# ParBLiSS/kmerind

Hardware: AMD Instinct MI355X
Metric: kmers_per_sec_indexed (higher is better)
Workload: dtype u64

## Files before the change

kmerind_amd/csrc/kmi_front.h:

```cpp
#pragma once
#include "kmi_front_bytes.h"

namespace kmi {

constexpr int kFrWaves = 4, kFrThreads = kFrWaves * kWave;
constexpr uint32_t kFrRing = 256;
constexpr uint32_t kFrRunQ = 256;
constexpr uint32_t kFrStep = 4096;
constexpr uint32_t kFrRowDw = 12;
constexpr uint32_t kFrNone = 0xffu;
constexpr uint32_t kFrOverrun = 256u << 10;

struct FrRange { uint32_t l0, n_lines, n_runs, n_items; };
struct __attribute__((packed, aligned(1))) FrU4 { uint32_t x, y, z, w; };

template <int W> struct FrCfg {
  static constexpr int SEG = W >= 19 ? 127 : (W >= 13 ? 80 : (W >= 11 ? 64 : 44));
  static constexpr int KMAX = W >= 19 ? 32 : (W >= 13 ? 28 : (W >= 11 ? 22 : 20));
  static constexpr int ND = (SEG + KMAX - 1 + 3) / 4;
  static constexpr int NR = (ND + 3) / 4;
};

__device__ __forceinline__ uint32_t pack_dna4(uint32_t w, uint32_t *ok_out = nullptr) {
  const uint32_t x = w & 0xDFDFDFDFu;
  const uint32_t idx = (x >> 1) & 0x03030303u;
  const uint32_t expect = byte_perm(0u, 0x47544341u, idx);
  const uint32_t ok = zero_bytes(x ^ expect);
  if (ok_out) *ok_out = ok;
  const uint32_t lut = byte_perm(0u, 0x01000203u, idx);
  const uint32_t v1 = ok >> 7, vm = v1 | (v1 << 1);
  const uint32_t cc = (lut & vm) | (0x03030303u & ~vm);
  const uint32_t p1 = cc | (cc >> 6);
  return (p1 | (p1 >> 12)) & 0xFFu;
}

__device__ __forceinline__ uint32_t dna4_ok(uint32_t w) {
  const uint32_t x = w & 0xDFDFDFDFu;
  const uint32_t idx = (x >> 1) & 0x03030303u;
  return zero_bytes(x ^ byte_perm(0u, 0x47544341u, idx));
}

#if defined(KMI_FR_TIMING) && !defined(KMI_FR_LEAVE)
#define KMI_FR_LEAVE
#endif
#ifdef KMI_FR_LEAVE
constexpr uint32_t kFrTimingWaves = 16384;
__device__ unsigned long long g_fr_wave_clock[2 * kFrTimingWaves];
#endif

template <int W, bool EDGES = false>
__global__ __launch_bounds__(kFrThreads) void sk_front_kernel(const uint8_t *__restrict__ bytes, uint64_t n_bytes, uint64_t range_bytes, uint32_t n_ranges,
                                                             uint32_t k, bool rna, uint32_t run_cap, uint32_t item_cap, uint32_t ranges_per_group,
                                                             FrRange *__restrict__ info, uint32_t *__restrict__ run_items, uint32_t *__restrict__ rows,
                                                             uint32_t *__restrict__ items, uint32_t *__restrict__ wg_hist,
                                                             unsigned long long *__restrict__ n_windows, uint32_t *__restrict__ flags,
                                                             uint32_t r_first = 0u, uint32_t r_end = 0xffffffffu, uint32_t *__restrict__ queue = nullptr) {
  constexpr bool edges = EDGES;
  if (r_end > n_ranges) r_end = n_ranges;
  using F = FrCfg<W>;
  constexpr int CAP = kSkListCap;
  constexpr uint32_t INF = 0xffffffffu, RM = kFrRing - 1u, QM = kFrRunQ - 1u;
  __shared__ uint32_t s_S[kFrWaves][kFrRing], s_E[kFrWaves][kFrRing], s_rq[kFrWaves][kFrRunQ];
  __shared__ uint32_t s_list[kFrWaves][(CAP + 2) * kWave];
  __shared__ uint32_t s_hist[kFrWaves][kNumCoarse];
  const uint32_t lane = lane_id(), wv = wave_id();
  uint32_t *const S = s_S[wv], *const E = s_E[wv], *const rq = s_rq[wv], *const list = s_list[wv], *const hist = s_hist[wv];
  auto wave_sync = [&]() { asm volatile("s_waitcnt lgkmcnt(0)" ::: "memory"); __builtin_amdgcn_wave_barrier(); };
  const uint32_t m = k - (uint32_t)W + 1u;
  const uint32_t mmask = (m >= 16u) ? 0xffffffffu : ((1u << (2u * m)) - 1u);
  const uint32_t topsh = 2u * m - 2u;
  const uint32_t nmax = sk_nmax_of(k) - (edges ? kSkEdgeWindows : 0u);
  const uint32_t seg = (uint32_t)F::SEG;
  const uint32_t n_waves = gridDim.x * (uint32_t)kFrWaves;
#ifdef KMI_FR_LEAVE
  const unsigned long long t_enter = wall_clock64();
#endif
#ifdef KMI_FR_TIMING
  unsigned long long acc[8] = {0, 0, 0, 0, 0, 0, 0, 0}, tq = clock64();
#define FQ_MARK(i) { const unsigned long long now_ = clock64(); acc[i] += now_ - tq; tq = now_; }
#else
#define FQ_MARK(i)
#endif
  for (uint32_t r = r_first + blockIdx.x * (uint32_t)kFrWaves + wv; r < r_end;) {
    const uint64_t B = (uint64_t)r * range_bytes;
    const uint32_t len = (uint32_t)((n_bytes - B < range_bytes) ? (n_bytes - B) : range_bytes);
    for (uint32_t i = lane; i < (uint32_t)kNumCoarse; i += kWave) hist[i] = 0;
    uint32_t why = 0; bool bail = false;
    uint32_t q_next = 0;
    if (queue && lane == 0) q_next = atomicAdd(queue, 1u);
    uint32_t carry = (B == 0) ? 1u : (is_eol((uint32_t)__builtin_amdgcn_readfirstlane((int)bytes[B - 1])) ? 1u : 0u);
    const uint32_t r_next = queue ? r_first + n_waves + (uint32_t)__builtin_amdgcn_readfirstlane((int)q_next) : r + n_waves;
    const uint32_t eoff = carry ? 0u : 1u;
    uint32_t n_starts = 0, n_ends = 0, n_owned = 0, done = 0, l0 = (r == 0) ? 0u : INF;
    if (r == 0 && __builtin_amdgcn_readfirstlane((int)bytes[0]) != (int)'@') { why |= 2u; bail = true; }
    uint32_t rq_head = 0, rq_tail = 0, run_count = 0, item_count = 0;
    unsigned long long windows = 0;
    uint32_t p = 0;
    bool producing = true;
    FrU4 n0, n1, n2, n3;
    n0.x = n0.y = n0.z = n0.w = 0; n1 = n0; n2 = n0; n3 = n0;
    if (B + 64ull * lane + 64 <= n_bytes) {
      const uint8_t *q = bytes + B + 64ull * lane;
      n0 = *reinterpret_cast<const FrU4 *>(q); n1 = *reinterpret_cast<const FrU4 *>(q + 16);
      n2 = *reinterpret_cast<const FrU4 *>(q + 32); n3 = *reinterpret_cast<const FrU4 *>(q + 48);
    }
    uint32_t mk_ch = 0, mk_want = 0;
    auto eol32 = [](const FrU4 &a, const FrU4 &b) -> uint32_t {
      uint32_t d0 = __builtin_amdgcn_udot4(eol_flags(a.x), 0x08040201u, 0u, false);
      d0 = __builtin_amdgcn_udot4(eol_flags(a.y), 0x80402010u, d0, false);
      uint32_t d1 = __builtin_amdgcn_udot4(eol_flags(a.z), 0x08040201u, 0u, false);
      d1 = __builtin_amdgcn_udot4(eol_flags(a.w), 0x80402010u, d1, false);
      uint32_t d2 = __builtin_amdgcn_udot4(eol_flags(b.x), 0x08040201u, 0u, false);
      d2 = __builtin_amdgcn_udot4(eol_flags(b.y), 0x80402010u, d2, false);
      uint32_t d3 = __builtin_amdgcn_udot4(eol_flags(b.z), 0x08040201u, 0u, false);
      d3 = __builtin_amdgcn_udot4(eol_flags(b.w), 0x80402010u, d3, false);
      return (d0 >> 7) | (d1 << 1) | (d2 << 9) | (d3 << 17);
    };
    while (!bail) {
      while (producing && rq_tail - rq_head < (uint32_t)kWave && !bail) {
        const uint64_t g = B + p + 64ull * lane;
        uint32_t eol_lo = 0, eol_hi = 0;
        const FrU4 v0 = n0, v1 = n1, v2 = n2, v3 = n3;
        {
          const uint64_t gn = g + kFrStep;
          if (gn + 64 <= n_bytes) {
            const uint8_t *q = bytes + gn;
            n0 = *reinterpret_cast<const FrU4 *>(q); n1 = *reinterpret_cast<const FrU4 *>(q + 16);
            n2 = *reinterpret_cast<const FrU4 *>(q + 32); n3 = *reinterpret_cast<const FrU4 *>(q + 48);
          }
        }
        FQ_MARK(0)
        if (g + 64 <= n_bytes) {
          eol_lo = eol32(v0, v1); eol_hi = eol32(v2, v3);
        } else {
#pragma unroll 1
          for (uint32_t i = 0; i < 64u; ++i) {
            const bool e = (g + i >= n_bytes) || is_eol(bytes[g + i]);
            if (i < 32u) eol_lo |= (e ? 1u : 0u) << i; else eol_hi |= (e ? 1u : 0u) << (i - 32u);
          }
        }
        FQ_MARK(1)
        const uint32_t prev = (uint32_t)__builtin_amdgcn_update_dpp((int)carry, (int)(eol_hi >> 31), 0x138 , 0xf, 0xf, false);
        const uint32_t before_lo = (eol_lo << 1) | prev, before_hi = (eol_hi << 1) | (eol_lo >> 31);
        uint32_t ls_lo = ~eol_lo & before_lo, ls_hi = ~eol_hi & before_hi, le_lo = eol_lo & ~before_lo, le_hi = eol_hi & ~before_hi;
        const uint32_t base = p + 64u * lane;
        const uint32_t ns = (uint32_t)__builtin_popcount(ls_lo) + (uint32_t)__builtin_popcount(ls_hi);
        const uint32_t ne = (uint32_t)__builtin_popcount(le_lo) + (uint32_t)__builtin_popcount(le_hi);
        if (__any(ns > 8u || ne > 8u)) { why |= 4u; bail = true; break; }
        const uint32_t no = base < len ? ns : 0u;
        const uint32_t packed = ns | (ne << 10) | (no << 20);
        const uint32_t inc = wave_inclusive_sum_dpp(packed);
        const uint32_t tot = __builtin_amdgcn_readlane(inc, kWave - 1);
        const uint32_t NS = tot & 1023u, NE = (tot >> 10) & 1023u, NO = tot >> 20;
        if (NS > kFrRing / 2u || NE > kFrRing / 2u) { why |= 4u; bail = true; break; }
        uint32_t rs = n_starts + ((inc - packed) & 1023u), re = n_ends + (((inc - packed) >> 10) & 1023u);
        while (ls_lo) { S[rs & RM] = base + (uint32_t)__builtin_ctz(ls_lo); ++rs; ls_lo &= ls_lo - 1u; }
        while (ls_hi) { S[rs & RM] = base + 32u + (uint32_t)__builtin_ctz(ls_hi); ++rs; ls_hi &= ls_hi - 1u; }
        while (le_lo) { E[re & RM] = base + (uint32_t)__builtin_ctz(le_lo); ++re; le_lo &= le_lo - 1u; }
        while (le_hi) { E[re & RM] = base + 32u + (uint32_t)__builtin_ctz(le_hi); ++re; le_hi &= le_hi - 1u; }
        n_starts += NS; n_ends += NE; n_owned += NO;
        carry = (uint32_t)__builtin_amdgcn_readlane(eol_hi, kWave - 1) >> 31;
        p += kFrStep;
        if (p > len + kFrOverrun) { why |= 32u; bail = true; break; }
        const bool at_eof = B + p > n_bytes;
        wave_sync();
        if (l0 == INF && n_starts > 0u) {
          if ((uint32_t)__builtin_amdgcn_readfirstlane((int)S[0]) >= len) l0 = kFrNone;
          else if (at_eof && n_starts < 6u) {
            l0 = (0u - n_starts) & 3u;
          } else if (n_starts >= 6u) {
            const uint32_t nl = 6u;
            uint32_t c = 0;
            if (lane < nl) c = bytes[B + S[lane]];
            const uint32_t c2 = __shfl_down(c, 2, kWave);
            const bool cand = lane < 4u && lane + 2u < nl && c == (uint32_t)'@' && c2 == (uint32_t)'+';
            const unsigned long long cm = __ballot(cand);
            if (__popcll(cm) != 1) { why |= 8u; bail = true; break; }
            l0 = (4u - (uint32_t)__builtin_ctzll(cm)) & 3u;
          }
        }
        if (l0 == kFrNone) { producing = false; break; }
        if (l0 != INF) {
          const uint32_t complete = n_ends >= eoff ? (n_starts < n_ends - eoff ? n_starts : n_ends - eoff) : 0u;
          for (uint32_t j0 = done; j0 < complete && !bail; j0 += kWave) {
            const uint32_t j = j0 + lane;
            const bool have = j < complete;
            uint32_t sj = 0, L = 0, role = 4;
            if (have) { sj = S[j & RM]; L = E[(j + eoff) & RM] - sj; role = (l0 + j) & 3u; }
            const bool owned = have && sj < len;
            bool bad = false;
            if (mk_want && mk_ch != mk_want) bad = true;
            mk_want = 0;
            if (owned && (role == 0u || role == 2u)) { mk_ch = bytes[B + sj]; mk_want = role == 0u ? (uint32_t)'@' : (uint32_t)'+'; }
            if (have && role == 3u && j >= 2u && S[(j - 2u) & RM] < len) bad = bad || (E[(j - 2u + eoff) & RM] - S[(j - 2u) & RM] != L);
            if (__any(bad)) {
              why |= 16u; bail = true; break;
            }
            uint32_t nr = 0, nwin = 0;
            if (owned && role == 1u && L >= k) { nwin = L - k + 1u; nr = (nwin + seg - 1u) / seg; }
            const uint32_t rinc = wave_inclusive_sum_dpp(nr);
            const uint32_t rtot = __builtin_amdgcn_readlane(rinc, kWave - 1);
            if ((rq_tail + rtot - rq_head > kFrRunQ || __any(have && (sj >> 24))) && rtot) { { why |= 32u; bail = true; break; } }
            uint32_t o = rq_tail + rinc - nr;
            for (uint32_t i = 0; i < nr; ++i) {
              const uint32_t left = nwin - i * seg;
              rq[(o + i) & QM] = (sj + i * seg) | (((left < seg ? left : seg) - 1u) << 24);
            }
            rq_tail += rtot;
          }
          if (bail) break;
          done = complete;
          if (at_eof || (p >= len && complete >= n_owned + 2u)) producing = false;
        } else if (at_eof) { producing = false; }
        wave_sync();
      }
      if (bail) break;
      FQ_MARK(2)
      const uint32_t avail = rq_tail - rq_head;
      if (avail == 0u) { if (!producing) break; continue; }
      const uint32_t take = avail < (uint32_t)kWave ? avail : (uint32_t)kWave;
      const bool mine = lane < take;
      const uint32_t rv = mine ? rq[(rq_head + lane) & QM] : 0u;
      rq_head += take;
      if (run_count + take > run_cap) { why |= 64u; bail = true; break; }
      const uint32_t L = mine ? (rv >> 24) + 1u : 0u;
      const uint64_t g0 = B + (rv & 0xffffffu);
      {
        const uint32_t wsum = __builtin_amdgcn_readlane(wave_inclusive_sum_dpp(L), kWave - 1);
        windows += wsum;
      }
      uint32_t rw[16];
#pragma unroll
      for (int i = 0; i < 16; ++i) rw[i] = 0;
      uint32_t other = 0;
      auto pack_exact = [&]() {
#pragma unroll
        for (int q = 0; q < F::NR; ++q) {
          FrU4 v = *reinterpret_cast<const FrU4 *>(bytes + g0 + 16 * q);
          if (rna) { v.x = swap_tu_dword(v.x); v.y = swap_tu_dword(v.y); v.z = swap_tu_dword(v.z); v.w = swap_tu_dword(v.w); }
          uint32_t okd[4];
          rw[q] = pack_dna4(v.x, &okd[0]) | (pack_dna4(v.y, &okd[1]) << 8) | (pack_dna4(v.z, &okd[2]) << 16) | (pack_dna4(v.w, &okd[3]) << 24);
          if (edges) {
            const uint32_t nbits = 8u * (L + k - 1u);
#pragma unroll
            for (int e = 0; e < 4; ++e) {
              const uint32_t at = 8u * (16u * (uint32_t)q + 4u * (uint32_t)e);
              const uint32_t vm = nbits >= at + 32u ? 0x80808080u : (nbits <= at ? 0u : (0x80808080u & ((1u << (nbits - at)) - 1u)));
              other |= ~okd[e] & vm;
            }
          }
        }
      };
      constexpr bool fast_pack = !edges;
      const bool whole = mine && g0 + 16ull * F::NR <= n_bytes;
      if (fast_pack) {
        uint32_t bad = 0;
        if (whole) {
          const uint32_t nb = L + k - 1u;
#pragma unroll
          for (int q = 0; q < F::NR; ++q) {
            FrU4 v = *reinterpret_cast<const FrU4 *>(bytes + g0 + 16 * q);
            if (rna) { v.x = swap_tu_dword(v.x); v.y = swap_tu_dword(v.y); v.z = swap_tu_dword(v.z); v.w = swap_tu_dword(v.w); }
            uint32_t d = 0;
            const uint32_t c0 = pack_codes4(v.x, d), c1 = pack_codes4(v.y, d), c2 = pack_codes4(v.z, d), c3 = pack_codes4(v.w, d);
            rw[q] = c0 | (c1 << 8) | (c2 << 16) | (c3 << 24);
            bad |= (16u * (uint32_t)(q + 1) <= nb) ? d : 0u;
          }
          const uint32_t rem = nb & 15u, qt = nb >> 4;
          if (rem) {
            FrU4 v = *reinterpret_cast<const FrU4 *>(bytes + g0 + 16u * qt);
            if (rna) { v.x = swap_tu_dword(v.x); v.y = swap_tu_dword(v.y); v.z = swap_tu_dword(v.z); v.w = swap_tu_dword(v.w); }
            bad |= dna4_other_in_first(v.x, rem) | dna4_other_in_first(v.y, rem > 4u ? rem - 4u : 0u) |
                   dna4_other_in_first(v.z, rem > 8u ? rem - 8u : 0u) | dna4_other_in_first(v.w, rem > 12u ? rem - 12u : 0u);
          }
          bad &= 0xDFDFDFDFu;
        }
        if (__any(bad != 0u)) { if (whole) pack_exact(); }
      } else if (whole) pack_exact();
      if (mine && !whole) {
        const uint32_t nb = L + k - 1u;
#pragma unroll 1
        for (uint32_t i = 0; i < nb; ++i) {
          uint32_t c = bytes[g0 + i];
          if (rna) c = swap_tu_dword(c) & 0xffu;
          const uint32_t code = pack_dna4(c | 0x0A0A0A00u) & 3u;
          if (edges) other |= ~dna4_ok(c | 0x41414100u) & 0x80u;
          const uint32_t wi = i >> 4, sh = (i & 15u) * 2u;
#pragma unroll
          for (int q = 0; q < F::NR; ++q) rw[q] |= (wi == (uint32_t)q) ? (code << sh) : 0u;
        }
      }
      if (edges) {
        if (mine) {
          const uint32_t nb = L + k - 1u;
          uint32_t lb = bytes[g0 - 1u], rb = g0 + nb < n_bytes ? (uint32_t)bytes[g0 + nb] : (uint32_t)'\n';
          if (rna) { lb = swap_tu_dword(lb) & 0xffu; rb = swap_tu_dword(rb) & 0xffu; }
          const uint32_t lc = is_eol(lb) ? 0u : 4u - (pack_dna4(lb | 0x0A0A0A00u) & 3u), rc = is_eol(rb) ? 0u : 4u - (pack_dna4(rb | 0x0A0A0A00u) & 3u);
          if (!is_eol(lb)) other |= ~dna4_ok(lb | 0x41414100u) & 0x80u;
          if (!is_eol(rb)) other |= ~dna4_ok(rb | 0x41414100u) & 0x80u;
          rw[kFrRowDw - 1] = lc | (rc << 3);
        }
        if (__any(other != 0u)) { why |= 1024u; bail = true; break; }
      }
      FQ_MARK(3)
      if (mine) {
        const uint64_t ri = (uint64_t)r * run_cap + run_count + lane;
        uint4 *rp = reinterpret_cast<uint4 *>(rows + ri * kFrRowDw);
        rp[0] = make_uint4(rw[0], rw[1], rw[2], rw[3]);
        rp[1] = make_uint4(rw[4], rw[5], rw[6], rw[7]);
        if (edges) rp[2] = make_uint4(rw[8], rw[9], rw[10], rw[11]);
        else *reinterpret_cast<uint2 *>(rp + 2) = make_uint2(rw[8], rw[9]);
      }
      uint32_t cnt = 0;
      {
        const uint32_t nblk = mine ? (L + (uint32_t)W - 2u) / (uint32_t)W + 1u : 0u;
        uint32_t R = rw[0] & mmask, Fw = sk_fwd_of(rw[0] & mmask, m);
        {
          const uint32_t sh0 = 2u * (m - 1u);
#pragma unroll
          for (int i = 0; i < F::NR; ++i) rw[i] = __builtin_amdgcn_alignbit(rw[i + 1], rw[i], sh0);
        }
        uint32_t sprev[W + 1];
#pragma unroll
        for (int j = 0; j <= W; ++j) sprev[j] = INF;
        const uint32_t a_first = (uint32_t)(uintptr_t)((lds_u32_t *)list + lane), a_stop = a_first + (uint32_t)CAP * 4u * kWave;
        uint32_t addr = a_first;
        uint32_t prevv = 0;
        const uint32_t nblk_max = (uint32_t)__builtin_amdgcn_readlane((int)wave_inclusive_max_dpp(nblk), kWave - 1);
        auto block = [&](auto first_block, uint32_t wbase ) {
          constexpr bool FIRST = decltype(first_block)::value;
          const uint32_t clo = rw[0], chi = rw[1];
          {
            constexpr int WS = (2 * W) / 32, BS = (2 * W) % 32;
#pragma unroll
            for (int i = 0; i < F::NR; ++i) rw[i] = __builtin_amdgcn_alignbit(rw[i + WS + 1], rw[i + WS], BS);
          }
          uint32_t hh[W];
          uint32_t pm = INF;
#pragma unroll
          for (int j = 0; j < W; ++j) {
            if (j > 0 || !FIRST) {
              const uint32_t c = (j < 16) ? ((clo >> (2 * (j & 15))) & 3u) : ((chi >> (2 * (j & 15))) & 3u);
              R = (R >> 2) | (c << topsh);
              Fw = ((Fw << 2) | (c ^ 3u)) & mmask;
            }
            const uint32_t h = sk_order_hash(R < Fw ? R : Fw);
            hh[j] = h;
            pm = pm < h ? pm : h;
            if (FIRST && j < W - 1) continue;
            const uint32_t sp = sprev[j + 1];
            const uint32_t curv = sp < pm ? sp : pm;
            const uint32_t wi = wbase + (uint32_t)j < 127u ? wbase + (uint32_t)j : 127u;
            *(lds_u32_t *)(uintptr_t)addr = (curv << 7) | wi;
            const uint32_t step = (FIRST || curv != prevv) ? 4u * kWave : 0u;
            addr = addr + step < a_stop ? addr + step : a_stop;
            prevv = curv;
          }
          sprev[W] = INF;
          sprev[W - 1] = hh[W - 1];
#pragma unroll
          for (int j = W - 2; j >= 0; --j) sprev[j] = hh[j] < sprev[j + 1] ? hh[j] : sprev[j + 1];
        };
        if (nblk_max) block(std::true_type{}, 0u - (uint32_t)(W - 1));
        for (uint32_t b = 1; b < nblk_max; ++b) block(std::false_type{}, b * (uint32_t)W - (uint32_t)(W - 1));
        cnt = (addr - a_first) / (4u * kWave);
      }
      FQ_MARK(4)
      if (__any(cnt >= (uint32_t)CAP)) { why |= 128u; bail = true; break; }
      list[cnt * kWave + lane] = cnt | 127u;
      wave_sync();
      const uint32_t cmax = (uint32_t)__builtin_amdgcn_readlane((int)wave_inclusive_max_dpp(cnt), kWave - 1);
      uint32_t jstar = cmax, head = 0;
      {
#define KMI_FR_TURN(J, CUR, NX)                                                                   \
        {                                                                                         \
          const uint32_t w0 = (CUR) & 127u, wn = (NX) & 127u;                                     \
          const bool valid = (J) < cnt && w0 < L;                                                 \
          const uint32_t n = (wn < L ? wn : L) - w0;  \
          if (__any(valid && n > nmax)) { jstar = (J); break; }                                   \
          if (!__any(valid)) break;                                                               \
          if (valid) {                                                                            \
            const uint32_t h27 = sk_bucket_bits27((CUR) >> 7);                                    \
            atomicAdd(&hist[h27 >> 19], 1u);                                                      \
            list[(J) * kWave + lane] = (n - 1u) | (h27 << 5);                                     \
            ++head;                                                                               \
          }                                                                                       \
        }
        uint32_t e0 = list[lane], e1 = list[kWave + lane];
        for (uint32_t j = 0; j < cmax; j += 2u) {
          const uint32_t e2 = list[(j + 2u) * kWave + lane], e3 = list[(j + 3u) * kWave + lane];
          KMI_FR_TURN(j, e0, e1)
          KMI_FR_TURN(j + 1u, e1, e2)
          e0 = e2; e1 = e3;
        }
#undef KMI_FR_TURN
      }
      uint32_t top = (uint32_t)CAP + 2u;
      if (jstar < cmax) {
        uint32_t nxt_w = L;
        uint32_t it_nx = list[(cmax - 1u) * kWave + lane];
        for (uint32_t jj = cmax; jj-- > jstar;) {
          const uint32_t it = it_nx;
          if (jj > jstar) it_nx = list[(jj - 1u) * kWave + lane];
          const uint32_t w0 = it & 127u;
          if (jj < cnt && w0 < L) {
            const uint32_t h27 = sk_bucket_bits27(it >> 7);
            uint32_t left = nxt_w - w0;
            nxt_w = w0;
            while (left) {
              uint32_t n = left;
              while (n > nmax) n -= nmax;
              left -= n;
              if (top <= jj || top <= 2u) { top = 0xffffffffu; left = 0; break; }
              --top;
              atomicAdd(&hist[h27 >> 19], 1u);
              list[top * kWave + lane] = (n - 1u) | (h27 << 5);
            }
            if (top == 0xffffffffu) break;
          }
        }
      }
      const uint32_t tail = (uint32_t)CAP + 2u - top;
      if (__any(head + tail > (uint32_t)CAP)) { why |= 128u; bail = true; break; }
      cnt = head + tail;
      FQ_MARK(5)
      const uint32_t cinc = wave_inclusive_sum_dpp(cnt);
      const uint32_t ctot = __builtin_amdgcn_readlane(cinc, kWave - 1);
      if (item_count + ctot > item_cap) { why |= 256u; bail = true; break; }
      if (mine) {
        const uint32_t ex = item_count + cinc - cnt;
        uint32_t *dst = items + (uint64_t)r * item_cap + ex;
        if (jstar == cmax) for (uint32_t j = 0; j < cnt; ++j) dst[j] = list[j * kWave + lane];
        else for (uint32_t j = 0; j < cnt; ++j) dst[j] = list[(j < head ? j : top + j - head) * kWave + lane];
        const uint64_t ri = (uint64_t)r * run_cap + run_count + lane;
        run_items[ri] = ex | (cnt << 26);
      }
      run_count += take;
      item_count += ctot;
      wave_sync();
      FQ_MARK(6)
    }
    if (!bail && __any(mk_want && mk_ch != mk_want)) { why |= 16u; bail = true; }
    if (bail) { if (lane == 0) { atomicOr(&flags[FLAG_SK_DECLINED], 4u); atomicOr(&flags[FLAG_SK_WHY], why); } }
    wave_sync();
    if (lane == 0) {
      FrRange fr; fr.l0 = (l0 == INF) ? kFrNone : l0; fr.n_lines = (l0 == INF || l0 == kFrNone) ? 0u : n_owned; fr.n_runs = run_count; fr.n_items = item_count;
      info[r] = fr;
      if (windows) atomicAdd(n_windows, windows);
    }
    const uint32_t grp = r / ranges_per_group;
    for (uint32_t i = lane; i < (uint32_t)kNumCoarse; i += kWave) {
      const uint32_t c = hist[i];
      if (c) atomicAdd(&wg_hist[(uint64_t)grp * kNumCoarse + i], c);
    }
    wave_sync();
    FQ_MARK(7)
    r = r_next;
  }
#ifdef KMI_FR_TIMING
  if (lane == 0) for (int i = 0; i < 8; ++i) atomicAdd(&reinterpret_cast<unsigned long long *>(flags + FLAG_CLOCKS)[i], acc[i]);
#endif
#ifdef KMI_FR_LEAVE
  if (lane == 0 && blockIdx.x * (uint32_t)kFrWaves + wv < kFrTimingWaves) {
    g_fr_wave_clock[2u * (blockIdx.x * (uint32_t)kFrWaves + wv)] = t_enter;
    g_fr_wave_clock[2u * (blockIdx.x * (uint32_t)kFrWaves + wv) + 1u] = wall_clock64();
  }
#endif
}

constexpr int kFrRowLds = 11;
constexpr uint32_t kFrMaxGroupRanges = 128;
constexpr int kFrScThreads = 512;
constexpr int kFrScItems = 7168;
template <bool CANON>
__global__ __launch_bounds__(kFrScThreads, 2) void sk_scatter_rows_kernel(const FrRange *__restrict__ info, uint32_t n_ranges, uint32_t rpg, uint32_t run_cap,
                                                                         uint32_t item_cap, uint32_t k, const uint32_t *__restrict__ run_items,
                                                                         const uint32_t *__restrict__ rows, const uint32_t *__restrict__ items,
                                                                         const uint64_t *__restrict__ wg_off, uint64_t *__restrict__ out, uint32_t lp,
                                                                         const uint32_t *__restrict__ flags, uint32_t edges = 0u) {
  if (__hip_atomic_load(&flags[FLAG_SK_DECLINED], __ATOMIC_RELAXED, __HIP_MEMORY_SCOPE_AGENT)) return;
  constexpr int NT = kFrScThreads, CAP = kSkListCap, ICAP = kFrScItems;
  static_assert(ICAP >= CAP, "a run's items must fit a round");
  __shared__ uint16_t s_stage[ICAP];
  __shared__ uint32_t s_items[ICAP + 4];
  __shared__ uint8_t s_xbits[ICAP];
  __shared__ uint32_t s_row[NT * kFrRowLds + 4];
  __shared__ uint32_t s_ibase[NT];
  __shared__ uint8_t s_runw[NT];
  __shared__ uint8_t s_runx[NT];
  __shared__ uint32_t s_cnt[kNumCoarse];
  __shared__ uint32_t s_cur[kNumCoarse];
  __shared__ uint64_t s_gbase[kNumCoarse];
  __shared__ uint32_t s_part[kNumCoarse / kWave];
  __shared__ uint32_t s_scan[NT / kWave + 2];
  __shared__ uint32_t s_pre[kFrMaxGroupRanges + 1];
  const bool bl = threadIdx.x < kNumCoarse;
  uint64_t cursor = bl ? wg_off[(uint64_t)blockIdx.x * kNumCoarse + threadIdx.x] : 0ull;
  if (bl) s_cnt[threadIdx.x] = 0;
  const uint32_t r_first = blockIdx.x * rpg;
  const uint32_t nr = r_first >= n_ranges ? 0u : (n_ranges - r_first < rpg ? n_ranges - r_first : rpg);
  if (threadIdx.x == 0) {
    uint32_t acc = 0;
    for (uint32_t q = 0; q < nr; ++q) { s_pre[q] = acc; acc += info[r_first + q].n_runs; }
    s_pre[nr] = acc;
  }
  lds_barrier();
  const uint32_t total_runs = s_pre[nr];
  const uint32_t *const g_items = items + (uint64_t)r_first * item_cap;
  for (uint32_t rb = 0; rb < total_runs;) {
    const uint32_t G = rb + threadIdx.x;
    uint32_t ri = 0, q = 0;
    uint64_t run = 0;
    if (G < total_runs) {
      static_assert(kFrMaxGroupRanges <= 128u, "seven probes");
#pragma unroll
      for (uint32_t step = 64u; step; step >>= 1) {
        const uint32_t t = q + step;
        if (t < nr && G >= s_pre[t]) q = t;
      }
      run = (uint64_t)(r_first + q) * run_cap + (G - s_pre[q]);
      ri = run_items[run];
    }
    uint32_t cnt = ri >> 26;
    uint32_t total;
    const uint32_t pre = block_exclusive_scan<uint32_t>(cnt, s_scan, &total);
    const bool taken = G < total_runs && pre + cnt <= (uint32_t)ICAP;
    const uint32_t n_taken = (uint32_t)__syncthreads_count(taken);
    if (!taken) cnt = 0;
    if (taken) {
      const uint4 *rp = reinterpret_cast<const uint4 *>(rows + run * kFrRowDw);
      const uint4 q0 = rp[0], q1 = rp[1], q2 = rp[2];
      uint32_t *row = s_row + threadIdx.x * kFrRowLds;
      row[0] = q0.x; row[1] = q0.y; row[2] = q0.z; row[3] = q0.w; row[4] = q1.x; row[5] = q1.y; row[6] = q1.z; row[7] = q1.w;
      row[8] = q2.x; row[9] = q2.y; row[10] = 0;
      if (edges) s_runx[threadIdx.x] = (uint8_t)q2.w;
      const uint32_t *src = g_items + (q * item_cap + (ri & 0x3ffffffu));
      uint32_t woff = 0;
#pragma unroll
      for (int v4 = 0; v4 < CAP / 4; ++v4) {
        if ((uint32_t)(4 * v4) < cnt) {
          const FrU4 v = *reinterpret_cast<const FrU4 *>(src + 4 * v4);
          const uint32_t it[4] = {v.x, v.y, v.z, v.w};
#pragma unroll
          for (int e = 0; e < 4; ++e)
            if ((uint32_t)(4 * v4 + e) < cnt) {
              const uint32_t n1 = it[e] & 31u, h27 = it[e] >> 5;
              s_items[pre + 4 * v4 + e] = woff | (n1 << 7) | ((h27 >> 7) << 12);
              s_xbits[pre + 4 * v4 + e] = (uint8_t)(h27 & 127u);
              atomicAdd(&s_cnt[h27 >> 19], 1u);
              woff += n1 + 1u;
            }
        }
      }
    }
    s_ibase[threadIdx.x] = pre;
    if (edges) {
      uint32_t wsum = 0;
      for (uint32_t j = 0; j < cnt; ++j) wsum += ((s_items[pre + j] >> 7) & 31u) + 1u;
      s_runw[threadIdx.x] = (uint8_t)wsum;
    }
    lds_barrier();
    uint32_t c = 0, inc = 0;
    if (bl) {
      c = s_cnt[threadIdx.x];
      s_cnt[threadIdx.x] = 0;
      inc = wave_inclusive_sum_dpp(c);
      if (lane_id() == kWave - 1) s_part[wave_id()] = inc;
    }
    lds_barrier();
    if (bl) {
      uint32_t wpre = 0;
#pragma unroll
      for (uint32_t w = 0; w < kNumCoarse / kWave; ++w) wpre += (w < wave_id()) ? s_part[w] : 0u;
      const uint32_t lo = wpre + inc - c;
      s_cur[threadIdx.x] = lo;
      s_gbase[threadIdx.x] = cursor - lo;
      cursor += c;
    }
    lds_barrier();
    for (uint32_t j = 0; j < cnt; ++j) {
      const uint32_t item = s_items[pre + j];
      s_stage[atomicAdd(&s_cur[item >> 24], 1u)] = (uint16_t)((threadIdx.x << 5) | j);
    }
    lds_barrier();
    const uint32_t n_items = pre + cnt;
    const uint32_t round_items = (uint32_t)__builtin_amdgcn_readfirstlane((int)s_cur[kNumCoarse - 1]);
    (void)n_items;
    for (uint32_t s = threadIdx.x; s < round_items; s += NT) {
      const uint32_t e = s_stage[s], rl = e >> 5, j = e & 31u;
      const uint32_t item = s_items[s_ibase[rl] + j];
      const uint32_t h27 = ((item >> 12) << 7) | (uint32_t)s_xbits[s_ibase[rl] + j], n1 = (item >> 7) & 31u;
      const uint32_t hs = ((h27 << lp) & 0x7ffffffu) >> 9;
      uint64_t w0, w1;
      bool flipped = false;
      sk_assemble_row<CANON>(s_row + rl * kFrRowLds, 2u * (item & 127u), k + n1, n1, hs, w0, w1, &flipped);
      if (edges) {
        const uint32_t *row = s_row + rl * kFrRowLds;
        const uint32_t wfirst = item & 127u, after = wfirst + n1 + k;
        auto cc = [&](uint32_t i) -> uint32_t { return (row[i >> 4] >> (2u * (i & 15u))) & 3u; };
        const uint32_t runx = s_runx[rl];
        const uint32_t lc = wfirst ? 1u + (3u - cc(wfirst - 1u)) : (runx & 7u);
        const uint32_t rc = wfirst + n1 + 1u < (uint32_t)s_runw[rl] ? 1u + (3u - cc(after)) : (runx >> 3);
        const uint32_t left = flipped ? (rc ? 5u - rc : 0u) : lc, right = flipped ? (lc ? 5u - lc : 0u) : rc;
        w1 |= ((uint64_t)(left | (right << 3)) << kRecEdgeShift) | ((uint64_t)(flipped ? 1u : 0u) << kRecFlipShift);
      }
      reinterpret_cast<ulonglong2 *>(out)[s_gbase[h27 >> 19] + s] = make_ulonglong2(w0, w1);
    }
    rb += n_taken;
    lds_barrier();
  }
}

__global__ __launch_bounds__(1024) void sk_front_verify_kernel(const FrRange *__restrict__ info, uint32_t n_ranges, uint32_t ranges_per_group,
                                                             uint64_t *__restrict__ group_runs ,
                                                             uint64_t *__restrict__ totals , uint32_t *__restrict__ flags) {
  __shared__ uint64_t s_scan[1024 / 64 + 2];
  __shared__ uint32_t s_bad;
  if (threadIdx.x == 0) s_bad = 0;
  lds_barrier();
  const uint32_t per = (n_ranges + 1023u) / 1024u;
  const uint32_t r_lo = threadIdx.x * per < n_ranges ? threadIdx.x * per : n_ranges, r_hi = r_lo + per < n_ranges ? r_lo + per : n_ranges;
  uint64_t my_lines = 0, my_runs = 0, my_its = 0;
  for (uint32_t r = r_lo; r < r_hi; ++r) {
    const FrRange fr = info[r];
    my_lines += fr.n_lines; my_runs += fr.n_runs; my_its += fr.n_items;
  }
  uint64_t carry = 0, runs = 0, its = 0;
  uint64_t before = block_exclusive_scan<uint64_t>(my_lines, s_scan, &carry);
  for (uint32_t r = r_lo; r < r_hi; ++r) {
    const FrRange fr = info[r];
    if (fr.l0 != kFrNone && fr.n_lines && ((uint32_t)before & 3u) != fr.l0) s_bad = 1;
    before += fr.n_lines;
  }
  (void)block_exclusive_scan<uint64_t>(my_runs, s_scan, &runs);
  (void)block_exclusive_scan<uint64_t>(my_its, s_scan, &its);
  lds_barrier();
  if (threadIdx.x == 0) {
    totals[0] = carry; totals[1] = runs; totals[2] = its;
    if (s_bad) atomicOr(&flags[FLAG_SK_DECLINED], 4u);
  }
  const uint32_t groups = (n_ranges + ranges_per_group - 1) / ranges_per_group;
  for (uint32_t g = threadIdx.x; g < groups; g += blockDim.x) {
    uint64_t s = 0;
    for (uint32_t r = g * ranges_per_group; r < (g + 1) * ranges_per_group && r < n_ranges; ++r) s += info[r].n_runs;
    group_runs[g] = s;
  }
}

}
```

Baseline: 191.2 billion.

## Merge start/end rings into one ends-only ring and process whole FASTQ records per lane

Replaces the separate line-start and line-end LDS rings with a single ring. By default it records only line ends and derives each start from the previous end, falling back to an interleaved start/end-pair mode (by redoing the range) when consecutive EOL bytes appear. Record parsing is restructured so each lane handles one 4-line FASTQ record, batched until enough records are pending, with partial-fit handling of the run queue. This is meant to cut LDS writes and per-line loop iterations, at the cost of a possible redo pass and more complex bookkeeping.

```diff
diff --git a/kmerind_amd/csrc/kmi_front.h b/kmerind_amd/csrc/kmi_front.h
--- a/kmerind_amd/csrc/kmi_front.h
+++ b/kmerind_amd/csrc/kmi_front.h
@@ -4,7 +4,18 @@
 namespace kmi {
 
 constexpr int kFrWaves = 4, kFrThreads = kFrWaves * kWave;
-constexpr uint32_t kFrRing = 256;
+constexpr uint32_t kFrRing = 512;
+constexpr uint32_t kFrStepLines = 128;
+constexpr uint32_t kFrPendEnds = kFrRing - kFrStepLines - 2u, kFrPendPairs = kFrRing / 2u - kFrStepLines;
+#ifndef KMI_FR_PASS_RECORDS
+#define KMI_FR_PASS_RECORDS 64
+#endif
+constexpr uint32_t kFrPassRecords = KMI_FR_PASS_RECORDS;
+#ifdef KMI_FR_PAIRS_ONLY
+constexpr bool kFrEndsOnly = false;
+#else
+constexpr bool kFrEndsOnly = true;
+#endif
 constexpr uint32_t kFrRunQ = 256;
 constexpr uint32_t kFrStep = 4096;
 constexpr uint32_t kFrRowDw = 12;
@@ -60,11 +71,11 @@
   using F = FrCfg<W>;
   constexpr int CAP = kSkListCap;
   constexpr uint32_t INF = 0xffffffffu, RM = kFrRing - 1u, QM = kFrRunQ - 1u;
-  __shared__ uint32_t s_S[kFrWaves][kFrRing], s_E[kFrWaves][kFrRing], s_rq[kFrWaves][kFrRunQ];
+  __shared__ uint32_t s_ring[kFrWaves][kFrRing], s_rq[kFrWaves][kFrRunQ];
   __shared__ uint32_t s_list[kFrWaves][(CAP + 2) * kWave];
   __shared__ uint32_t s_hist[kFrWaves][kNumCoarse];
-  const uint32_t lane = lane_id(), wv = wave_id();
-  uint32_t *const S = s_S[wv], *const E = s_E[wv], *const rq = s_rq[wv], *const list = s_list[wv], *const hist = s_hist[wv];
+  const uint32_t lane = lane_id(), wv = (uint32_t)__builtin_amdgcn_readfirstlane((int)wave_id());
+  uint32_t *const Rg = s_ring[wv], *const rq = s_rq[wv], *const list = s_list[wv], *const hist = s_hist[wv];
   auto wave_sync = [&]() { asm volatile("s_waitcnt lgkmcnt(0)" ::: "memory"); __builtin_amdgcn_wave_barrier(); };
   const uint32_t m = k - (uint32_t)W + 1u;
   const uint32_t mmask = (m >= 16u) ? 0xffffffffu : ((1u << (2u * m)) - 1u);
@@ -84,14 +95,19 @@
   for (uint32_t r = r_first + blockIdx.x * (uint32_t)kFrWaves + wv; r < r_end;) {
     const uint64_t B = (uint64_t)r * range_bytes;
     const uint32_t len = (uint32_t)((n_bytes - B < range_bytes) ? (n_bytes - B) : range_bytes);
+    uint32_t q_next = 0;
+    if (queue && lane == 0) q_next = atomicAdd(queue, 1u);
+    const uint32_t carry0 = (B == 0) ? 1u : (is_eol((uint32_t)__builtin_amdgcn_readfirstlane((int)bytes[B - 1])) ? 1u : 0u);
+    const uint32_t r_next = queue ? r_first + n_waves + (uint32_t)__builtin_amdgcn_readfirstlane((int)q_next) : r + n_waves;
+    const uint32_t eoff = carry0 ? 0u : 1u;
+    bool simple = kFrEndsOnly;
+    for (;;) {
+    bool redo = false;
     for (uint32_t i = lane; i < (uint32_t)kNumCoarse; i += kWave) hist[i] = 0;
     uint32_t why = 0; bool bail = false;
-    uint32_t q_next = 0;
-    if (queue && lane == 0) q_next = atomicAdd(queue, 1u);
-    uint32_t carry = (B == 0) ? 1u : (is_eol((uint32_t)__builtin_amdgcn_readfirstlane((int)bytes[B - 1])) ? 1u : 0u);
-    const uint32_t r_next = queue ? r_first + n_waves + (uint32_t)__builtin_amdgcn_readfirstlane((int)q_next) : r + n_waves;
-    const uint32_t eoff = carry ? 0u : 1u;
-    uint32_t n_starts = 0, n_ends = 0, n_owned = 0, done = 0, l0 = (r == 0) ? 0u : INF;
+    uint32_t carry = carry0;
+    uint32_t n_starts = 0, n_ends = 0, n_owned = 0, done = 0, complete = 0, l0 = (r == 0) ? 0u : INF;
+    bool fin = false;
     if (r == 0 && __builtin_amdgcn_readfirstlane((int)bytes[0]) != (int)'@') { why |= 2u; bail = true; }
     uint32_t rq_head = 0, rq_tail = 0, run_count = 0, item_count = 0;
     unsigned long long windows = 0;
@@ -104,7 +120,8 @@
       n0 = *reinterpret_cast<const FrU4 *>(q); n1 = *reinterpret_cast<const FrU4 *>(q + 16);
       n2 = *reinterpret_cast<const FrU4 *>(q + 32); n3 = *reinterpret_cast<const FrU4 *>(q + 48);
     }
-    uint32_t mk_ch = 0, mk_want = 0;
+    uint32_t mk_hd = (uint32_t)'@', mk_plus = (uint32_t)'+';
+    auto line_start = [&](uint32_t j) -> uint32_t { return simple ? (j + eoff ? Rg[(j + eoff - 1u) & RM] + 1u : 0u) : Rg[(2u * j) & RM]; };
     auto eol32 = [](const FrU4 &a, const FrU4 &b) -> uint32_t {
       uint32_t d0 = __builtin_amdgcn_udot4(eol_flags(a.x), 0x08040201u, 0u, false);
       d0 = __builtin_amdgcn_udot4(eol_flags(a.y), 0x80402010u, d0, false);
@@ -118,8 +135,10 @@
     };
     while (!bail) {
       while (producing && rq_tail - rq_head < (uint32_t)kWave && !bail) {
+       if (!fin && !(l0 != INF && ((complete - done + ((l0 + done) & 3u)) >> 2) >= kFrPassRecords) &&
+           n_starts - done <= (simple ? kFrPendEnds : kFrPendPairs)) {
         const uint64_t g = B + p + 64ull * lane;
-        uint32_t eol_lo = 0, eol_hi = 0;
+        uint32_t eol_lo = 0, eol_hi = 0, in_lo = 0xffffffffu, in_hi = 0xffffffffu;
         const FrU4 v0 = n0, v1 = n1, v2 = n2, v3 = n3;
         {
           const uint64_t gn = g + kFrStep;
@@ -133,16 +152,20 @@
         if (g + 64 <= n_bytes) {
           eol_lo = eol32(v0, v1); eol_hi = eol32(v2, v3);
         } else {
+          in_lo = in_hi = 0;
 #pragma unroll 1
           for (uint32_t i = 0; i < 64u; ++i) {
-            const bool e = (g + i >= n_bytes) || is_eol(bytes[g + i]);
-            if (i < 32u) eol_lo |= (e ? 1u : 0u) << i; else eol_hi |= (e ? 1u : 0u) << (i - 32u);
+            const bool in = g + i < n_bytes;
+            const bool e = !in || is_eol(bytes[g + i]);
+            if (i < 32u) { eol_lo |= (e ? 1u : 0u) << i; in_lo |= (in ? 1u : 0u) << i; }
+            else { eol_hi |= (e ? 1u : 0u) << (i - 32u); in_hi |= (in ? 1u : 0u) << (i - 32u); }
           }
         }
         FQ_MARK(1)
         const uint32_t prev = (uint32_t)__builtin_amdgcn_update_dpp((int)carry, (int)(eol_hi >> 31), 0x138 , 0xf, 0xf, false);
         const uint32_t before_lo = (eol_lo << 1) | prev, before_hi = (eol_hi << 1) | (eol_lo >> 31);
-        uint32_t ls_lo = ~eol_lo & before_lo, ls_hi = ~eol_hi & before_hi, le_lo = eol_lo & ~before_lo, le_hi = eol_hi & ~before_hi;
+        if (simple && __any(((eol_lo & before_lo & in_lo) | (eol_hi & before_hi & in_hi)) != 0u)) { redo = true; bail = true; break; }
+        const uint32_t ls_lo = ~eol_lo & before_lo, ls_hi = ~eol_hi & before_hi, le_lo = eol_lo & ~before_lo, le_hi = eol_hi & ~before_hi;
         const uint32_t base = p + 64u * lane;
         const uint32_t ns = (uint32_t)__builtin_popcount(ls_lo) + (uint32_t)__builtin_popcount(ls_hi);
         const uint32_t ne = (uint32_t)__builtin_popcount(le_lo) + (uint32_t)__builtin_popcount(le_hi);
@@ -152,12 +175,23 @@
         const uint32_t inc = wave_inclusive_sum_dpp(packed);
         const uint32_t tot = __builtin_amdgcn_readlane(inc, kWave - 1);
         const uint32_t NS = tot & 1023u, NE = (tot >> 10) & 1023u, NO = tot >> 20;
-        if (NS > kFrRing / 2u || NE > kFrRing / 2u) { why |= 4u; bail = true; break; }
+        if (NS > kFrStepLines || NE > kFrStepLines) { why |= 4u; bail = true; break; }
         uint32_t rs = n_starts + ((inc - packed) & 1023u), re = n_ends + (((inc - packed) >> 10) & 1023u);
-        while (ls_lo) { S[rs & RM] = base + (uint32_t)__builtin_ctz(ls_lo); ++rs; ls_lo &= ls_lo - 1u; }
-        while (ls_hi) { S[rs & RM] = base + 32u + (uint32_t)__builtin_ctz(ls_hi); ++rs; ls_hi &= ls_hi - 1u; }
-        while (le_lo) { E[re & RM] = base + (uint32_t)__builtin_ctz(le_lo); ++re; le_lo &= le_lo - 1u; }
-        while (le_hi) { E[re & RM] = base + 32u + (uint32_t)__builtin_ctz(le_hi); ++re; le_hi &= le_hi - 1u; }
+        unsigned long long le = ((unsigned long long)le_hi << 32) | le_lo;
+        if (simple) {
+          while (__any(le != 0ull)) {
+            if (le) { Rg[re & RM] = base + (uint32_t)__builtin_ctzll(le); ++re; le &= le - 1ull; }
+          }
+        } else {
+          unsigned long long ls = ((unsigned long long)ls_hi << 32) | ls_lo;
+          while (__any((ls | le) != 0ull)) {
+            if (ls) { Rg[(2u * rs) & RM] = base + (uint32_t)__builtin_ctzll(ls); ++rs; ls &= ls - 1ull; }
+            if (le) {
+              if (re >= eoff) Rg[(2u * (re - eoff) + 1u) & RM] = base + (uint32_t)__builtin_ctzll(le);
+              ++re; le &= le - 1ull;
+            }
+          }
+        }
         n_starts += NS; n_ends += NE; n_owned += NO;
         carry = (uint32_t)__builtin_amdgcn_readlane(eol_hi, kWave - 1) >> 31;
         p += kFrStep;
@@ -165,13 +199,13 @@
         const bool at_eof = B + p > n_bytes;
         wave_sync();
         if (l0 == INF && n_starts > 0u) {
-          if ((uint32_t)__builtin_amdgcn_readfirstlane((int)S[0]) >= len) l0 = kFrNone;
+          if ((uint32_t)__builtin_amdgcn_readfirstlane((int)line_start(0u)) >= len) l0 = kFrNone;
           else if (at_eof && n_starts < 6u) {
             l0 = (0u - n_starts) & 3u;
           } else if (n_starts >= 6u) {
             const uint32_t nl = 6u;
             uint32_t c = 0;
-            if (lane < nl) c = bytes[B + S[lane]];
+            if (lane < nl) c = bytes[B + line_start(lane)];
             const uint32_t c2 = __shfl_down(c, 2, kWave);
             const bool cand = lane < 4u && lane + 2u < nl && c == (uint32_t)'@' && c2 == (uint32_t)'+';
             const unsigned long long cm = __ballot(cand);
@@ -180,40 +214,67 @@
           }
         }
         if (l0 == kFrNone) { producing = false; break; }
-        if (l0 != INF) {
-          const uint32_t complete = n_ends >= eoff ? (n_starts < n_ends - eoff ? n_starts : n_ends - eoff) : 0u;
-          for (uint32_t j0 = done; j0 < complete && !bail; j0 += kWave) {
-            const uint32_t j = j0 + lane;
-            const bool have = j < complete;
-            uint32_t sj = 0, L = 0, role = 4;
-            if (have) { sj = S[j & RM]; L = E[(j + eoff) & RM] - sj; role = (l0 + j) & 3u; }
-            const bool owned = have && sj < len;
-            bool bad = false;
-            if (mk_want && mk_ch != mk_want) bad = true;
-            mk_want = 0;
-            if (owned && (role == 0u || role == 2u)) { mk_ch = bytes[B + sj]; mk_want = role == 0u ? (uint32_t)'@' : (uint32_t)'+'; }
-            if (have && role == 3u && j >= 2u && S[(j - 2u) & RM] < len) bad = bad || (E[(j - 2u + eoff) & RM] - S[(j - 2u) & RM] != L);
-            if (__any(bad)) {
-              why |= 16u; bail = true; break;
-            }
-            uint32_t nr = 0, nwin = 0;
-            if (owned && role == 1u && L >= k) { nwin = L - k + 1u; nr = (nwin + seg - 1u) / seg; }
-            const uint32_t rinc = wave_inclusive_sum_dpp(nr);
-            const uint32_t rtot = __builtin_amdgcn_readlane(rinc, kWave - 1);
-            if ((rq_tail + rtot - rq_head > kFrRunQ || __any(have && (sj >> 24))) && rtot) { { why |= 32u; bail = true; break; } }
-            uint32_t o = rq_tail + rinc - nr;
+        if (l0 == INF) {
+          if (at_eof) producing = false;
+          wave_sync();
+          continue;
+        }
+        complete = n_ends >= eoff ? (n_starts < n_ends - eoff ? n_starts : n_ends - eoff) : 0u;
+        fin = at_eof || (p >= len && complete >= n_owned + 2u);
+       }
+        const uint32_t jb = done - ((l0 + done) & 3u);
+        const uint32_t whole = (complete - jb) >> 2;
+        if (!fin && whole < kFrPassRecords && n_starts - done <= (simple ? kFrPendEnds : kFrPendPairs)) { wave_sync(); continue; }
+        if (fin && done == complete) { producing = false; break; }
+        const uint32_t ahead = fin ? complete - jb : 4u * whole;
+        const uint32_t lim = jb + (ahead < 4u * kWave ? ahead : 4u * kWave);
+        const uint32_t n_rec = (lim - jb + 3u) >> 2;
+        if (n_rec == 0u) { why |= 32u; bail = true; break; }
+        {
+          const uint32_t jr = jb + 4u * lane;
+          const bool in_pass = lane < n_rec;
+          uint32_t s[4], e[4];
+          bool v[4];
+#pragma unroll
+          for (uint32_t t = 0; t < 4u; ++t) v[t] = in_pass && (int32_t)(jr + t - done) >= 0 && (int32_t)(lim - (jr + t)) > 0;
+          if (simple) {
+            uint32_t x[5];
+#pragma unroll
+            for (uint32_t t = 0; t < 5u; ++t) x[t] = Rg[(jr + eoff - 1u + t) & RM];
+#pragma unroll
+            for (uint32_t t = 0; t < 4u; ++t) { s[t] = (jr + t + eoff) ? x[t] + 1u : 0u; e[t] = x[t + 1u]; }
+          } else {
+#pragma unroll
+            for (uint32_t t = 0; t < 4u; ++t) { s[t] = Rg[(2u * (jr + t)) & RM]; e[t] = Rg[(2u * (jr + t) + 1u) & RM]; }
+          }
+          const bool own_hd = v[0] && s[0] < len, own_seq = v[1] && s[1] < len, own_plus = v[2] && s[2] < len;
+          bool bad = mk_hd != (uint32_t)'@' || mk_plus != (uint32_t)'+';
+          mk_hd = (uint32_t)'@'; mk_plus = (uint32_t)'+';
+          if (own_hd) mk_hd = bytes[B + s[0]];
+          if (own_plus) mk_plus = bytes[B + s[2]];
+          const uint32_t L = e[1] - s[1];
+          if (v[3] && own_seq) bad = bad || (e[3] - s[3] != L);
+          if (__any(bad)) { why |= 16u; bail = true; break; }
+          uint32_t nr = 0, nwin = 0;
+          if (own_seq && L >= k) { nwin = L - k + 1u; nr = (nwin + seg - 1u) / seg; }
+          const uint32_t rinc = wave_inclusive_sum_dpp(nr);
+          const uint32_t n_fit = (uint32_t)__popcll(__ballot(in_pass && rinc <= kFrRunQ - (rq_tail - rq_head)));
+          if (n_fit == 0u || __any(nr && (s[1] >> 24))) { why |= 32u; bail = true; break; }
+          if (lane < n_fit) {
+            const uint32_t o = rq_tail + rinc - nr;
             for (uint32_t i = 0; i < nr; ++i) {
               const uint32_t left = nwin - i * seg;
-              rq[(o + i) & QM] = (sj + i * seg) | (((left < seg ? left : seg) - 1u) << 24);
+              rq[(o + i) & QM] = (s[1] + i * seg) | (((left < seg ? left : seg) - 1u) << 24);
             }
-            rq_tail += rtot;
-          }
-          if (bail) break;
-          done = complete;
-          if (at_eof || (p >= len && complete >= n_owned + 2u)) producing = false;
-        } else if (at_eof) { producing = false; }
+          }
+          rq_tail += (uint32_t)__builtin_amdgcn_readlane((int)rinc, (int)(n_fit - 1u));
+          done = n_fit == n_rec ? lim : jb + 4u * n_fit;
+        }
+        if (fin && done == complete) producing = false;
         wave_sync();
-      }
+        FQ_MARK(2)
+      }
+      if (redo) break;
       if (bail) break;
       FQ_MARK(2)
       const uint32_t avail = rq_tail - rq_head;
@@ -440,7 +501,8 @@
       wave_sync();
       FQ_MARK(6)
     }
-    if (!bail && __any(mk_want && mk_ch != mk_want)) { why |= 16u; bail = true; }
+    if (redo) { simple = false; wave_sync(); continue; }
+    if (!bail && __any(mk_hd != (uint32_t)'@' || mk_plus != (uint32_t)'+')) { why |= 16u; bail = true; }
     if (bail) { if (lane == 0) { atomicOr(&flags[FLAG_SK_DECLINED], 4u); atomicOr(&flags[FLAG_SK_WHY], why); } }
     wave_sync();
     if (lane == 0) {
@@ -455,6 +517,8 @@
     }
     wave_sync();
     FQ_MARK(7)
+    break;
+    }
     r = r_next;
   }
 #ifdef KMI_FR_TIMING
```

Result: faster. 197.5 billion (median of 6 runs) (+3.3%).
